# nghiapq77/face-recognition-cpp-tensorrt

Measured on AMD Instinct MI355X. Metric: faces/sec end-to-end (detect+embed+match), 640x640 batch=32, 1M gallery, higher is better.
Workload: dtype f16 MFMA recogniser convs (fp32 accumulate) + fp32-accurate detector (fp32 MFMA, fp16 hi/lo-split MFMA for the 64-channel 3x3 convs) + int8-screened coarse scan (fp16 MFMA on exactly widened int8 rows) + exact f32 re-rank match (bit-identical to the exact f32 scan)

## Files before the change

### face-recognition-cpp-tensorrt_amd/csrc/kernels_arc_c64.hip

```cpp
#include <cstdlib>

#include "frt_kernels.h"

namespace {

constexpr int SW = 56;
constexpr int PW = SW + 2;
constexpr int PROWB = 144;
constexpr int NDMA = (4 * PW * 9 + 127) / 128;
constexpr int PATCH_B = NDMA * 2 * 1024;
constexpr int RING = 5;
constexpr int EROW = 36;

template <int MODE>
__global__ __launch_bounds__(128) void conv64_kernel(ConvMfmaArgs p, int n_strips) {
    extern __shared__ __attribute__((aligned(16))) char smem[];
    char *patch = smem;
    float *etile = reinterpret_cast<float *>(smem + 2 * PATCH_B);
    const int tid = threadIdx.x, lane = tid & 63, cb = tid >> 6;
    const int r = lane & 31, hi = lane >> 5;
    const int H = p.H, W = p.W;
    const int strips_x = W / SW, strips_per_img = (H / 2) * strips_x;

    const int nwg = gridDim.x;
    const int bq = nwg >> 3, brem = nwg & 7;
    const int xcd = blockIdx.x & 7, slot = blockIdx.x >> 3;
    const int wid = (xcd < brem ? xcd * (bq + 1) : brem * (bq + 1) + (xcd - brem) * bq) + slot;
    const int k_full = n_strips / nwg, rem_strips = n_strips - k_full * nwg;
    auto strip_of = [&](int k) {
        if (k < k_full) return wid + k * nwg;
        return (k == k_full && (int)blockIdx.x < rem_strips) ? k_full * nwg + (int)blockIdx.x : n_strips;
    };

    half8 wreg[9][4];
    {
        const half_t *wrow = p.w + (long)(cb * 32 + r) * 576 + 8 * hi;
#pragma unroll
        for (int tap = 0; tap < 9; ++tap)
#pragma unroll
            for (int kk = 0; kk < 4; ++kk) wreg[tap][kk] = *reinterpret_cast<const half8 *>(wrow + tap * 64 + kk * 16);
    }
    const int ec0 = cb * 32 + (lane & 3) * 8;
    float q0[8], q1[8], q2[8], q3[8];
#pragma unroll
    for (int e = 0; e < 8; ++e) {
        q0[e] = p.p0[ec0 + e];
        q1[e] = MODE == EPI_PRELU ? 0.f : p.p1[ec0 + e];
        q2[e] = (MODE == EPI_BN_ADD_BN && p.out1) ? p.p2[ec0 + e] : 0.f;
        q3[e] = (MODE == EPI_BN_ADD_BN && p.out1) ? p.p3[ec0 + e] : 0.f;
    }

    int bbase[4];
#pragma unroll
    for (int t = 0; t < 4; ++t) {
        const int q = 32 * t + r;
        const int qq = q < 2 * SW ? q : 0;
        const int row = qq / SW, col = qq - row * SW;
        bbase[t] = (row * PW + col) * PROWB + hi * 16;
    }

    unsigned prel[NDMA];
#pragma unroll
    for (int q = 0; q < NDMA; ++q) {
        const int slot = (2 * q + cb) * 64 + lane;
        const int pix = slot / 9, part = slot - pix * 9;
        const int pr = pix / PW, pc = pix - pr * PW;
        const bool dead = part == 8 || pix >= 4 * PW;
        const unsigned need = dead ? 16u : ((pr == 0 ? 1u : 0u) | (pr == 3 ? 2u : 0u) | (pc == 0 ? 4u : 0u) | (pc == PW - 1 ? 8u : 0u));
        const unsigned rel = dead ? 0u : (unsigned)((pr * W + pc) * 64 + part * 8);
        prel[q] = rel | (need << 27);
    }
    auto issue_patch = [&](int strip, char *dst) {
        const int b = strip / strips_per_img, rem = strip - b * strips_per_img;
        const int sy = rem / strips_x, sx = rem - sy * strips_x;
        const int y0 = sy * 2 - 1, x0 = sx * SW - 1;
        const unsigned edge = 16u | (y0 < 0 ? 1u : 0u) | (y0 + 3 >= H ? 2u : 0u) | (x0 < 0 ? 4u : 0u) | (x0 + PW - 1 >= W ? 8u : 0u);
        const half_t *win = p.x + ((long)b * H * W + (long)y0 * W + x0) * 64;
#pragma unroll
        for (int q = 0; q < NDMA; ++q) {
            const bool live = ((prel[q] >> 27) & edge) == 0;
            const half_t *src = live ? win + (prel[q] & 0x7ffffffu) : p.zeros;
            __builtin_amdgcn_global_load_lds((const __attribute__((address_space(1))) void *)src,
                                             (__attribute__((address_space(3))) void *)(dst + (2 * q + cb) * 1024), 16, 0, 0);
        }
    };

    int k = 0;
    int strip = strip_of(0);
    if (strip >= n_strips) return;
    issue_patch(strip, patch);
    asm volatile("s_waitcnt vmcnt(0)" ::: "memory");
    __syncthreads();
    int cur = 0;

    float *et = etile + cb * 32 * EROW;
    for (;;) {
        const int next = strip_of(k + 1);
        const bool has_next = next < n_strips;
        if (has_next) issue_patch(next, patch + (cur ^ 1) * PATCH_B);
        half8 scv[4][2];
        if (MODE == EPI_BN_ADD_BN) {
            const int b = strip / strips_per_img, rem = strip - b * strips_per_img;
            const int sy = rem / strips_x, sx = rem - sy * strips_x;
#pragma unroll
            for (int t = 0; t < 4; ++t)
#pragma unroll
                for (int i = 0; i < 2; ++i) {
                    const int q = 32 * t + (lane >> 2) + 16 * i;
                    const int qq = q < 2 * SW ? q : 0;
                    const int row = qq / SW, col = qq - row * SW;
                    const long m = (long)b * H * W + (long)(sy * 2 + row) * W + sx * SW + col;
                    scv[t][i] = *reinterpret_cast<const half8 *>(p.sc + m * 64 + ec0);
                }
        }

        floatx16 acc[4];
#pragma unroll
        for (int t = 0; t < 4; ++t)
#pragma unroll
            for (int e = 0; e < 16; ++e) acc[t][e] = 0.f;

        const char *pb = patch + cur * PATCH_B;
        half8 bf[RING][4];
        auto read_b = [&](int s, half8 (&dst)[4]) {
            const int tap = s >> 2, kk = s & 3;
            const int kh = tap / 3, kw = tap - kh * 3;
            const int off = (kh * PW + kw) * PROWB + kk * 32;
#pragma unroll
            for (int t = 0; t < 4; ++t) dst[t] = *reinterpret_cast<const half8 *>(pb + bbase[t] + off);
        };
#pragma unroll
        for (int s = 0; s < RING - 1; ++s)
            read_b(s, bf[s]);
#pragma unroll
        for (int s = 0; s < 36; ++s) {
            if (s + RING - 1 < 36) read_b(s + RING - 1, bf[(s + RING - 1) % RING]);
            __builtin_amdgcn_sched_barrier(0);
#pragma unroll
            for (int t = 0; t < 4; ++t) acc[t] = __builtin_amdgcn_mfma_f32_32x32x16_f16(wreg[s >> 2][s & 3], bf[s % RING][t], acc[t], 0, 0, 0);
            __builtin_amdgcn_sched_barrier(0);
        }

        asm volatile("s_waitcnt vmcnt(0)" ::: "memory");
        const int b = strip / strips_per_img, rem = strip - b * strips_per_img;
        const int sy = rem / strips_x, sx = rem - sy * strips_x;
        const long img_base = (long)b * H * W;
#pragma unroll
        for (int t = 0; t < 4; ++t) {
#pragma unroll
            for (int g = 0; g < 4; ++g) {
                floatx4 v = {acc[t][4 * g], acc[t][4 * g + 1], acc[t][4 * g + 2], acc[t][4 * g + 3]};
                *reinterpret_cast<floatx4 *>(et + r * EROW + 8 * g + 4 * hi) = v;
            }
#pragma unroll
            for (int i = 0; i < 2; ++i) {
                const int px = (lane >> 2) + 16 * i;
                const floatx4 v0 = *reinterpret_cast<const floatx4 *>(et + px * EROW + (lane & 3) * 8);
                const floatx4 v1 = *reinterpret_cast<const floatx4 *>(et + px * EROW + (lane & 3) * 8 + 4);
                const int q = 32 * t + px;
                if (q >= 2 * SW) continue;
                const int row = q / SW, col = q - row * SW;
                const long m = img_base + (long)(sy * 2 + row) * W + sx * SW + col;
                float v[8] = {v0[0], v0[1], v0[2], v0[3], v1[0], v1[1], v1[2], v1[3]};
                if (MODE == EPI_PRELU) {
#pragma unroll
                    for (int e = 0; e < 8; ++e) v[e] = v[e] > 0.f ? v[e] : v[e] * q0[e];
                } else {
#pragma unroll
                    for (int e = 0; e < 8; ++e) v[e] = v[e] * q0[e] + q1[e];
                }
                if (MODE == EPI_BN_ADD_BN) {
#pragma unroll
                    for (int e = 0; e < 8; ++e) v[e] += (float)scv[t][i][e];
                }
                half8 o;
#pragma unroll
                for (int e = 0; e < 8; ++e) o[e] = (half_t)v[e];
                *reinterpret_cast<half8 *>(p.out0 + m * 64 + ec0) = o;
                if (MODE == EPI_BN_ADD_BN && p.out1) {
                    half8 z;
#pragma unroll
                    for (int e = 0; e < 8; ++e) z[e] = (half_t)(v[e] * q2[e] + q3[e]);
                    *reinterpret_cast<half8 *>(p.out1 + m * 64 + ec0) = z;
                }
            }
        }
        if (!has_next) break;
        __syncthreads();
        cur ^= 1;
        strip = next;
        ++k;
    }
}



template <int MODE>
void launch_c64_t(const ConvMfmaArgs &a, const ConvPlan &, hipStream_t s) {
    const int n_strips = a.B * (a.H / 2) * (a.W / SW);
    int grid = 512;
    if (grid > n_strips) grid = n_strips;
    const size_t lds = 2 * PATCH_B + 2 * 32 * EROW * sizeof(float);
    static bool attr_done[FRT_MAX_DEVICES] = {};
    if (frt_first_use_on_device(attr_done))
        (void)hipFuncSetAttribute(reinterpret_cast<const void *>(&conv64_kernel<MODE>), hipFuncAttributeMaxDynamicSharedMemorySize, (int)lds);
    hipLaunchKernelGGL((conv64_kernel<MODE>), dim3(grid), dim3(128), lds, s, a, n_strips);
}

const ConvRow kC64[] = {
    {"conv64_kernel<0>", launch_c64_t<EPI_PRELU>, -1},
    {"conv64_kernel<1>", launch_c64_t<EPI_BN>, -1},
    {"conv64_kernel<2>", launch_c64_t<EPI_BN_ADD_BN>, -1},
};

}

bool plan_c64(const ConvMfmaArgs &a, ConvPlan &p) {
    if (a.Cin != 64 || a.Cout != 64 || a.ks != 3 || a.stride != 1 || a.pad != 1 || a.Ho != a.H || a.Wo != a.W) return false;
    if ((a.H & 1) || a.W % SW || a.mode == EPI_PARTIAL) return false;
    if (a.mode == EPI_BN_ADD_BN && !(a.sc && a.sc_stride == 1 && a.sc_h == a.H && a.sc_w == a.W)) return false;
    conv_plan_row(p, CONV_C64, kC64, a.mode == EPI_PRELU ? 0 : (a.mode == EPI_BN ? 1 : 2));
    return true;
}

void launch_c64(const ConvMfmaArgs &a, const ConvPlan &p, hipStream_t s) { kC64[p.row].launch(a, p, s); }
```

Measured before the change: 43570.

## Software-pipeline c64 conv epilogue and DMA issue into MFMA stream

Splits each strip's 128-pixel accumulation into two halves. The epilogue of one half (LDS transpose, BN/PReLU, residual add, fp16 stores) is interleaved op by op between the MFMAs of the other half, including across strips. Next-strip global-to-LDS DMA issue and shortcut loads are also spread through the MFMA loop using raw inline asm, with precomputed offsets and a partial vmcnt wait in place of a full barrier drain. This targets the exposed serial epilogue and DMA issue latency, at the cost of much more complex scheduling, more live registers, and fragile hand-tuned waitcnt counts.

Measured after the change: 44290, median of 6. 1.6% higher.

```diff
diff --git a/face-recognition-cpp-tensorrt_amd/csrc/kernels_arc_c64.hip b/face-recognition-cpp-tensorrt_amd/csrc/kernels_arc_c64.hip
--- a/face-recognition-cpp-tensorrt_amd/csrc/kernels_arc_c64.hip
+++ b/face-recognition-cpp-tensorrt_amd/csrc/kernels_arc_c64.hip
@@ -1,4 +1,5 @@
 #include <cstdlib>
+#include <type_traits>
 
 #include "frt_kernels.h"
 
@@ -11,6 +12,22 @@
 constexpr int PATCH_B = NDMA * 2 * 1024;
 constexpr int RING = 5;
 constexpr int EROW = 36;
+constexpr int STEPS = 36;
+constexpr int GAPS = 2 * STEPS;
+
+template <int LO, int HI, class F>
+__device__ __forceinline__ void static_for(F &&f) {
+    if constexpr (LO < HI) {
+        f(std::integral_constant<int, LO>{});
+        static_for<LO + 1, HI>(f);
+    }
+}
+
+template <int MODE>
+struct DrainOps {
+    static constexpr int PER = (MODE == EPI_BN_ADD_BN ? 16 : 8) + 1;
+    static constexpr int count(int h) { return 12 + (h == 0 ? 4 : 3) * PER; }
+};
 
 template <int MODE>
 __global__ __launch_bounds__(128) void conv64_kernel(ConvMfmaArgs p, int n_strips) {
@@ -46,9 +63,10 @@
     for (int e = 0; e < 8; ++e) {
         q0[e] = p.p0[ec0 + e];
         q1[e] = MODE == EPI_PRELU ? 0.f : p.p1[ec0 + e];
-        q2[e] = (MODE == EPI_BN_ADD_BN && p.out1) ? p.p2[ec0 + e] : 0.f;
-        q3[e] = (MODE == EPI_BN_ADD_BN && p.out1) ? p.p3[ec0 + e] : 0.f;
-    }
+        q2[e] = (MODE == EPI_BN_ADD_BN && p.out1) ? p.p2[ec0 + e] : 1.f;
+        q3[e] = (MODE == EPI_BN_ADD_BN && p.out1) ? p.p3[ec0 + e] : -0.f;
+    }
+    half_t *const out1 = (MODE == EPI_BN_ADD_BN && p.out1) ? p.out1 : p.out0;
 
     int bbase[4];
 #pragma unroll
@@ -58,6 +76,12 @@
         const int row = qq / SW, col = qq - row * SW;
         bbase[t] = (row * PW + col) * PROWB + hi * 16;
     }
+    const int lane_off = (lane >> 2) * 64 + ec0;
+    const int lane_off11 = lane_off + ((lane >> 2) >= SW - 48 ? (W - SW) * 64 : 0);
+    auto group_off = [&](int h, int j, int i) __attribute__((always_inline)) {
+        const int q0s = 64 * h + 32 * j + 16 * i;
+        return (unsigned)(((h == 0 && j == 1 && i == 1) ? lane_off11 : lane_off) + (q0s + (q0s >= SW ? W - SW : 0)) * 64);
+    };
 
     unsigned prel[NDMA];
 #pragma unroll
@@ -66,131 +90,150 @@
         const int pix = slot / 9, part = slot - pix * 9;
         const int pr = pix / PW, pc = pix - pr * PW;
         const bool dead = part == 8 || pix >= 4 * PW;
-        const unsigned need = dead ? 16u : ((pr == 0 ? 1u : 0u) | (pr == 3 ? 2u : 0u) | (pc == 0 ? 4u : 0u) | (pc == PW - 1 ? 8u : 0u));
-        const unsigned rel = dead ? 0u : (unsigned)((pr * W + pc) * 64 + part * 8);
-        prel[q] = rel | (need << 27);
-    }
-    auto issue_patch = [&](int strip, char *dst) {
+        const unsigned need = 32u | (dead ? 16u : ((pr == 0 ? 1u : 0u) | (pr == 3 ? 2u : 0u) | (pc == 0 ? 4u : 0u) | (pc == PW - 1 ? 8u : 0u)));
+        const unsigned rel = dead ? 0u : (unsigned)((pr * W + pc) * 128 + part * 16);
+        prel[q] = rel | (need << 26);
+    }
+    struct Strip {
+        long pix0;
+        const char *win;
+        unsigned edge;
+    };
+    auto decode = [&](int strip, bool valid) __attribute__((always_inline)) {
         const int b = strip / strips_per_img, rem = strip - b * strips_per_img;
         const int sy = rem / strips_x, sx = rem - sy * strips_x;
         const int y0 = sy * 2 - 1, x0 = sx * SW - 1;
-        const unsigned edge = 16u | (y0 < 0 ? 1u : 0u) | (y0 + 3 >= H ? 2u : 0u) | (x0 < 0 ? 4u : 0u) | (x0 + PW - 1 >= W ? 8u : 0u);
-        const half_t *win = p.x + ((long)b * H * W + (long)y0 * W + x0) * 64;
-#pragma unroll
-        for (int q = 0; q < NDMA; ++q) {
-            const bool live = ((prel[q] >> 27) & edge) == 0;
-            const half_t *src = live ? win + (prel[q] & 0x7ffffffu) : p.zeros;
-            __builtin_amdgcn_global_load_lds((const __attribute__((address_space(1))) void *)src,
-                                             (__attribute__((address_space(3))) void *)(dst + (2 * q + cb) * 1024), 16, 0, 0);
+        Strip s;
+        s.pix0 = (long)b * H * W + (long)(sy * 2) * W + sx * SW;
+        s.win = reinterpret_cast<const char *>(p.x + (s.pix0 - W - 1) * 64);
+        s.edge = 16u | (valid ? 0u : 32u) | (y0 < 0 ? 1u : 0u) | (y0 + 3 >= H ? 2u : 0u) | (x0 < 0 ? 4u : 0u) | (x0 + PW - 1 >= W ? 8u : 0u);
+        return s;
+    };
+    const unsigned patch_lds = (unsigned)(size_t)(__attribute__((address_space(3))) char *)patch + __builtin_amdgcn_readfirstlane(cb) * 1024;
+    auto dma_src = [&](int q, const Strip &s) __attribute__((always_inline)) {
+        const bool live = ((prel[q] >> 26) & s.edge) == 0;
+        return live ? s.win + (prel[q] & 0x3ffffffu) : reinterpret_cast<const char *>(p.zeros);
+    };
+    auto dma_issue = [&](int q, const char *src, int buf) __attribute__((always_inline)) {
+        asm volatile("s_mov_b32 m0, %0\n\ts_nop 0\n\tglobal_load_lds_dwordx4 %1, off" ::"s"(patch_lds + buf * PATCH_B + q * 2048), "v"(src) : "memory");
+    };
+
+    int k = 0;
+    if (strip_of(0) >= n_strips) return;
+    Strip cs = decode(strip_of(0), true), ns = cs;
+    long prev_pix0 = 0;
+    bool has_next = false;
+#pragma unroll
+    for (int q = 0; q < NDMA; ++q) dma_issue(q, dma_src(q, cs), 0);
+    asm volatile("s_waitcnt vmcnt(0)" ::: "memory");
+    __builtin_amdgcn_s_barrier();
+    int cur = 0;
+
+    float *et = etile + cb * 32 * EROW;
+    floatx16 acc[2][2];
+    half8 scv[2][2][2];
+    floatx4 vb[2][2][2];
+    half8 oy, oz;
+
+    auto drain_op = [&](auto hc, auto nc, floatx16 (&a)[2], long pix0) __attribute__((always_inline)) {
+        constexpr int h = decltype(hc)::value, n = decltype(nc)::value, PER = DrainOps<MODE>::PER;
+        if constexpr (n < 12) {
+            constexpr int j = n / 6, w = n % 6;
+            if constexpr (w < 4) {
+                floatx4 v = {a[j][4 * w], a[j][4 * w + 1], a[j][4 * w + 2], a[j][4 * w + 3]};
+                *reinterpret_cast<floatx4 *>(et + r * EROW + 8 * w + 4 * hi) = v;
+            } else {
+                constexpr int i = w - 4;
+                const int px = (lane >> 2) + 16 * i;
+                vb[j][i][0] = *reinterpret_cast<const floatx4 *>(et + px * EROW + (lane & 3) * 8);
+                vb[j][i][1] = *reinterpret_cast<const floatx4 *>(et + px * EROW + (lane & 3) * 8 + 4);
+            }
+        } else {
+            constexpr int grp = (n - 12) / PER, w = (n - 12) % PER, j = grp >> 1, i = grp & 1;
+            static_assert(!(h == 1 && j == 1 && i == 1), "pixels 112..127 are never drained");
+            if constexpr (w < 8) {
+                constexpr int e = w;
+                float v = vb[j][i][e >> 2][e & 3];
+                if (MODE == EPI_PRELU) v = v > 0.f ? v : v * q0[e];
+                else v = v * q0[e] + q1[e];
+                if (MODE == EPI_BN_ADD_BN) v += (float)scv[h][j][i][e];
+                asm("" : "+v"(v));
+                oy[e] = (half_t)v;
+                vb[j][i][e >> 2][e & 3] = v;
+            } else if constexpr (w < PER - 1) {
+                constexpr int e = w - 8;
+                float z = vb[j][i][e >> 2][e & 3] * q2[e] + q3[e];
+                asm("" : "+v"(z));
+                oz[e] = (half_t)z;
+            } else {
+                const unsigned off = group_off(h, j, i);
+                *reinterpret_cast<half8 *>((p.out0 + pix0 * 64) + off) = oy;
+                if (MODE == EPI_BN_ADD_BN) *reinterpret_cast<half8 *>((out1 + pix0 * 64) + off) = oz;
+            }
         }
     };
-
-    int k = 0;
-    int strip = strip_of(0);
-    if (strip >= n_strips) return;
-    issue_patch(strip, patch);
-    asm volatile("s_waitcnt vmcnt(0)" ::: "memory");
-    __syncthreads();
-    int cur = 0;
-
-    float *et = etile + cb * 32 * EROW;
-    for (;;) {
+    auto drain = [&](auto hc, auto lo, auto hi_, floatx16 (&a)[2], long pix0) __attribute__((always_inline)) {
+        static_for<decltype(lo)::value, decltype(hi_)::value>([&](auto nc) __attribute__((always_inline)) { drain_op(hc, nc, a, pix0); });
+    };
+    auto load_sc = [&](int h, int j, int i, long pix0) __attribute__((always_inline)) {
+        scv[h][j][i] = *reinterpret_cast<const half8 *>((p.sc + pix0 * 64) + group_off(h, j, i));
+    };
+
+    auto strip_body = [&](auto first) __attribute__((always_inline)) {
         const int next = strip_of(k + 1);
-        const bool has_next = next < n_strips;
-        if (has_next) issue_patch(next, patch + (cur ^ 1) * PATCH_B);
-        half8 scv[4][2];
-        if (MODE == EPI_BN_ADD_BN) {
-            const int b = strip / strips_per_img, rem = strip - b * strips_per_img;
-            const int sy = rem / strips_x, sx = rem - sy * strips_x;
-#pragma unroll
-            for (int t = 0; t < 4; ++t)
-#pragma unroll
-                for (int i = 0; i < 2; ++i) {
-                    const int q = 32 * t + (lane >> 2) + 16 * i;
-                    const int qq = q < 2 * SW ? q : 0;
-                    const int row = qq / SW, col = qq - row * SW;
-                    const long m = (long)b * H * W + (long)(sy * 2 + row) * W + sx * SW + col;
-                    scv[t][i] = *reinterpret_cast<const half8 *>(p.sc + m * 64 + ec0);
-                }
-        }
-
-        floatx16 acc[4];
-#pragma unroll
-        for (int t = 0; t < 4; ++t)
-#pragma unroll
-            for (int e = 0; e < 16; ++e) acc[t][e] = 0.f;
-
+        has_next = next < n_strips;
+        ns = decode(next, has_next);
+        const char *src = nullptr;
         const char *pb = patch + cur * PATCH_B;
-        half8 bf[RING][4];
-        auto read_b = [&](int s, half8 (&dst)[4]) {
+        half8 bf[RING][2];
+        auto read_b = [&](int u, half8 (&d)[2]) __attribute__((always_inline)) {
+            const int h = u / STEPS, s = u - h * STEPS;
             const int tap = s >> 2, kk = s & 3;
             const int kh = tap / 3, kw = tap - kh * 3;
             const int off = (kh * PW + kw) * PROWB + kk * 32;
 #pragma unroll
-            for (int t = 0; t < 4; ++t) dst[t] = *reinterpret_cast<const half8 *>(pb + bbase[t] + off);
+            for (int j = 0; j < 2; ++j) d[j] = *reinterpret_cast<const half8 *>(pb + bbase[2 * h + j] + off);
         };
 #pragma unroll
-        for (int s = 0; s < RING - 1; ++s)
-            read_b(s, bf[s]);
-#pragma unroll
-        for (int s = 0; s < 36; ++s) {
-            if (s + RING - 1 < 36) read_b(s + RING - 1, bf[(s + RING - 1) % RING]);
+        for (int u = 0; u < RING - 1; ++u) read_b(u, bf[u]);
+        static_for<0, 2 * STEPS>([&](auto uc) __attribute__((always_inline)) {
+            constexpr int u = decltype(uc)::value, h = u / STEPS, s = u - h * STEPS;
+            if constexpr (u + RING - 1 < 2 * STEPS) read_b(u + RING - 1, bf[(u + RING - 1) % RING]);
             __builtin_amdgcn_sched_barrier(0);
-#pragma unroll
-            for (int t = 0; t < 4; ++t) acc[t] = __builtin_amdgcn_mfma_f32_32x32x16_f16(wreg[s >> 2][s & 3], bf[s % RING][t], acc[t], 0, 0, 0);
-            __builtin_amdgcn_sched_barrier(0);
-        }
-
-        asm volatile("s_waitcnt vmcnt(0)" ::: "memory");
-        const int b = strip / strips_per_img, rem = strip - b * strips_per_img;
-        const int sy = rem / strips_x, sx = rem - sy * strips_x;
-        const long img_base = (long)b * H * W;
-#pragma unroll
-        for (int t = 0; t < 4; ++t) {
-#pragma unroll
-            for (int g = 0; g < 4; ++g) {
-                floatx4 v = {acc[t][4 * g], acc[t][4 * g + 1], acc[t][4 * g + 2], acc[t][4 * g + 3]};
-                *reinterpret_cast<floatx4 *>(et + r * EROW + 8 * g + 4 * hi) = v;
-            }
-#pragma unroll
-            for (int i = 0; i < 2; ++i) {
-                const int px = (lane >> 2) + 16 * i;
-                const floatx4 v0 = *reinterpret_cast<const floatx4 *>(et + px * EROW + (lane & 3) * 8);
-                const floatx4 v1 = *reinterpret_cast<const floatx4 *>(et + px * EROW + (lane & 3) * 8 + 4);
-                const int q = 32 * t + px;
-                if (q >= 2 * SW) continue;
-                const int row = q / SW, col = q - row * SW;
-                const long m = img_base + (long)(sy * 2 + row) * W + sx * SW + col;
-                float v[8] = {v0[0], v0[1], v0[2], v0[3], v1[0], v1[1], v1[2], v1[3]};
-                if (MODE == EPI_PRELU) {
-#pragma unroll
-                    for (int e = 0; e < 8; ++e) v[e] = v[e] > 0.f ? v[e] : v[e] * q0[e];
+            static_for<0, 2>([&](auto jc) __attribute__((always_inline)) {
+                constexpr int j = decltype(jc)::value;
+                constexpr int g = 2 * s + j;
+                const floatx16 zero = {0.f, 0.f, 0.f, 0.f, 0.f, 0.f, 0.f, 0.f, 0.f, 0.f, 0.f, 0.f, 0.f, 0.f, 0.f, 0.f};
+                acc[h][j] = __builtin_amdgcn_mfma_f32_32x32x16_f16(wreg[s >> 2][s & 3], bf[u % RING][j], s == 0 ? zero : acc[h][j], 0, 0, 0);
+                __builtin_amdgcn_sched_barrier(0);
+                if constexpr (MODE == EPI_BN_ADD_BN && g < 8 && !(g & 1) && !(h == 1 && g == 6)) load_sc(h, g >> 2, (g >> 1) & 1, cs.pix0);
+                if constexpr (h == 0) {
+                    if constexpr (!(g & 1) && (g >> 1) < NDMA) src = dma_src(g >> 1, ns);
+                    if constexpr ((g & 1) && (g >> 1) < NDMA) dma_issue(g >> 1, src, cur ^ 1);
+                    constexpr int N = DrainOps<MODE>::count(1);
+                    if constexpr (!decltype(first)::value)
+                        drain(std::integral_constant<int, 1>{}, std::integral_constant<int, g * N / GAPS>{}, std::integral_constant<int, (g + 1) * N / GAPS>{}, acc[1], prev_pix0);
                 } else {
-#pragma unroll
-                    for (int e = 0; e < 8; ++e) v[e] = v[e] * q0[e] + q1[e];
+                    constexpr int N = DrainOps<MODE>::count(0);
+                    drain(std::integral_constant<int, 0>{}, std::integral_constant<int, g * N / GAPS>{}, std::integral_constant<int, (g + 1) * N / GAPS>{}, acc[0], cs.pix0);
                 }
-                if (MODE == EPI_BN_ADD_BN) {
-#pragma unroll
-                    for (int e = 0; e < 8; ++e) v[e] += (float)scv[t][i][e];
-                }
-                half8 o;
-#pragma unroll
-                for (int e = 0; e < 8; ++e) o[e] = (half_t)v[e];
-                *reinterpret_cast<half8 *>(p.out0 + m * 64 + ec0) = o;
-                if (MODE == EPI_BN_ADD_BN && p.out1) {
-                    half8 z;
-#pragma unroll
-                    for (int e = 0; e < 8; ++e) z[e] = (half_t)(v[e] * q2[e] + q3[e]);
-                    *reinterpret_cast<half8 *>(p.out1 + m * 64 + ec0) = z;
-                }
-            }
-        }
-        if (!has_next) break;
-        __syncthreads();
+                __builtin_amdgcn_sched_barrier(0);
+            });
+        });
+        if (MODE == EPI_BN_ADD_BN) asm volatile("s_waitcnt vmcnt(8)" ::: "memory");
+        else asm volatile("s_waitcnt vmcnt(4)" ::: "memory");
+        __builtin_amdgcn_s_barrier();
+    };
+
+    strip_body(std::true_type{});
+    while (has_next) {
+        prev_pix0 = cs.pix0;
+        cs = ns;
         cur ^= 1;
-        strip = next;
         ++k;
-    }
+        strip_body(std::false_type{});
+    }
+    drain(std::integral_constant<int, 1>{}, std::integral_constant<int, 0>{}, std::integral_constant<int, DrainOps<MODE>::count(1)>{}, acc[1], cs.pix0);
 }
 
 
```
